# phandasm/waveform

Hardware: AMD Instinct MI355X
Metric: spectra/sec at FFT=4096, batch=4096 streams; achieved HBM GB/s vs peak (higher is better)
Workload: dtype f32

## Files before the change

waveform_amd/csrc/wf_hip_plan.hip:

```cpp
#include <hip/hip_runtime.h>

#include <algorithm>
#include <cmath>
#include <cstdarg>
#include <cstdio>
#include <cstdlib>
#include <cstring>
#include <new>
#include <string>
#include <vector>

#include "wf_hip_internal.hpp"
#include "wf_geometry.hpp"

namespace wf::host {

thread_local std::string g_create_error;

int fail(wf_hip *h, int code, const char *fmt, ...)
{
    char buf[512];
    va_list ap;
    va_start(ap, fmt);
    vsnprintf(buf, sizeof(buf), fmt, ap);
// ... 111 lines not shown
    h->out_ch = h->tab.output_channels;
    h->disp_ch = h->tab.display_channels;
    h->num_bars = (uint32_t)h->tab.num_bars;
    h->ring_cap = next_pow2(ring_frames ? std::max(ring_frames, h->N) : std::max(2 * h->N, 4096u));
    h->plan = wf::plan_transform(cfg, ov);
    h->tick.mr.passes = h->plan.passes;
    std::copy(h->plan.radix, h->plan.radix + 4, h->tick.mr.radix);
    h->wave = cfg.waveform != 0;
    h->meter = cfg.meter != 0;
    if(h->wave) {
        h->M = h->N;
        h->ring_cap = next_pow2(std::max(ring_frames, 2 * (wave_samples + h->N)));
    }
    uint32_t pad = h->ring_cap >= 65536u ? 16448u : 0u;
#ifdef WF_DEV_BUILD
    if(const char *e = std::getenv("WF_HIP_RING_PAD"))
        pad = (uint32_t)std::strtoul(e, nullptr, 10) & ~3u;
#endif
    h->ring_stride = h->ring_cap + pad;
    if(h->wave)
        fill_wave_args(h, wave_samples);
    return WF_HIP_OK;
}

int open_device(wf_hip *h, int *cu_count)
{
    WF_HIP_TRY(h, hipSetDevice(h->device));
    hipDeviceProp_t prop{};
    WF_HIP_TRY(h, hipGetDeviceProperties(&prop, h->device));
    if(std::strncmp(prop.gcnArchName, "gfx950", 6) != 0)
        return fail(h, WF_HIP_ERR_NO_DEVICE, "device %d is %s; this library contains gfx950 code only", h->device, prop.gcnArchName);
    *cu_count = prop.multiProcessorCount;
    WF_HIP_TRY(h, hipStreamCreateWithFlags(&h->stream, hipStreamNonBlocking));
    WF_HIP_TRY(h, hipEventCreate(&h->ev0));
    WF_HIP_TRY(h, hipEventCreate(&h->ev1));
    return WF_HIP_OK;
}

size_t spectra(const wf_hip *h) { return (size_t)h->n_streams * h->cap_ch; }

int finish_create(wf_hip *h)
{
    WF_TRY_RC(wf_hip_reset(h, 0, h->n_streams));
    WF_HIP_TRY(h, hipStreamSynchronize(h->stream));
    return WF_HIP_OK;
}

int create_waveform(wf_hip *h)
{
    WF_TRY_RC(dev_alloc(h, &h->d_cend, (size_t)h->n_streams));
    WF_TRY_RC(dev_alloc(h, &h->d_wts, (size_t)h->n_streams));
    WF_TRY_RC(dev_alloc(h, &h->d_decibels, (size_t)h->n_streams * h->out_ch * h->M));
    WF_TRY_RC(dev_alloc(h, &h->d_flags, (size_t)h->n_streams));
    h->kernel_name = "waveform_tick_kernel";
    return finish_create(h);
}

int create_meter(wf_hip *h)
{
    WF_TRY_RC(dev_alloc(h, &h->d_mend, (size_t)h->n_streams));
    WF_TRY_RC(dev_alloc(h, &h->d_meter_buf, spectra(h)));
    WF_TRY_RC(dev_alloc(h, &h->d_meter_val, spectra(h)));
    WF_TRY_RC(dev_alloc(h, &h->d_flags, (size_t)h->n_streams));
    WF_TRY_RC(dev_alloc(h, &h->d_bars, spectra(h)));
    h->kernel_name = "meter_tick_kernel";
    fill_meter_args(h);
    return finish_create(h);
}

int alloc_spectrum_state(wf_hip *h)
{
    const wf_config *cfg = &h->cfg;
    WF_TRY_RC(dev_alloc(h, &h->d_tsmooth, spectra(h) * h->M));
    WF_TRY_RC(dev_alloc(h, &h->d_decibels, (size_t)h->n_streams * h->out_ch * h->M));
    h->flag_bufs = h->plan.want_split ? 3 : 1;
    WF_TRY_RC(dev_alloc(h, &h->d_flags, (size_t)h->flag_bufs * h->n_streams));
    if(h->plan.want_split)
        WF_TRY_RC(dev_alloc(h, &h->d_verdict, 3 * spectra(h)));
    if(h->num_bars)
        WF_TRY_RC(dev_alloc(h, &h->d_bars, (size_t)h->n_streams * h->disp_ch * h->num_bars));
    if(h->num_bars && cfg->mirror_freq_axis)
        WF_TRY_RC(dev_alloc(h, &h->d_bars_pre, (size_t)h->n_streams * h->disp_ch));
#ifdef WF_PHASE_TIMING
    WF_TRY_RC(dev_alloc(h, &h->tick.phase_clock, spectra(h) * 16));
#endif
    if(!cfg->vertices)
        return WF_HIP_OK;
    if(cfg->vertices > 3u || (cfg->vertices == 3u && (!cfg->bars || cfg->step_width < 1 || cfg->step_gap < 0)) || (cfg->vertices == 2u && cfg->bars) ||
       (!cfg->bars && !cfg->curve))
        return fail(h, WF_HIP_ERR_INVALID, "cfg.vertices: 1 needs bars or curve, 2 the curve, 3 bars with step_width >= 1 and step_gap >= 0");
    wf::VertexTables vtab;
    if(h->num_bars != 0)
        wf::build_vertex_tables(*cfg, (int)h->num_bars, vtab);
    if(h->num_bars != 0 && vtab.per_row > 0) {
        const size_t rows = (size_t)h->n_streams * h->disp_ch;
        float *d_cap_xy = nullptr;
        WF_TRY_RC(dev_alloc(h, &h->d_vert_counts, rows));
        WF_HIP_TRY(h, hipMemsetAsync(h->d_vert_counts, 0, rows * sizeof(uint32_t), h->stream));
        WF_TRY_RC(dev_alloc(h, &h->d_verts, rows * vtab.per_row));
        WF_HIP_TRY(h, hipMemsetAsync(h->d_verts, 0, rows * vtab.per_row * sizeof(wf::f4), h->stream));
        WF_TRY_RC(upload(h, &d_cap_xy, vtab.cap_xy));
        WF_HIP_TRY(h, hipStreamSynchronize(h->stream));
        fill_vertex_args(h, vtab, d_cap_xy);
    }
    return WF_HIP_OK;
}

int upload_window_tables(wf_hip *h)
{
    const std::vector<float> ones_m(h->M, 1.0f);
    const float in_scale = h->plan.in_scale;
    std::vector<float> win_dev(h->N, in_scale);
    for(size_t i = 0; i < h->tab.window.size() && i < win_dev.size(); ++i)
        win_dev[i] = h->tab.window[i] * in_scale;
    WF_TRY_RC(upload(h, &h->tick.window, win_dev));
    WF_TRY_RC(upload(h, &h->tick.slope, h->tab.slope.empty() ? ones_m : h->tab.slope));
    WF_HIP_TRY(h, hipStreamSynchronize(h->stream));
    return upload(h, &h->tick.rolloff, h->tab.rolloff);
}

struct DisplayRoom {
    bool own_kernel;
    size_t lds_floats;
    int threads, points, kmax;
};

void fill_bar_scalars(wf_hip *h)
{
    wf::BarArgs &b = h->tick.bar;
    b.gauss_radius = h->tab.gauss_radius;
    b.entries = (int)h->tab.bar_coef.size();
    b.num_bars = (int)h->num_bars;
    b.mirror = h->cfg.mirror_freq_axis ? 1 : 0;
    b.border_top = h->tab.border_top;
    b.border_bottom = h->tab.border_bottom;
    b.ceiling = (float)h->cfg.ceiling_db;
    b.dbrange = (float)(h->cfg.ceiling_db - h->cfg.floor_db);
    b.inv_dbrange = 1.0f / b.dbrange;
    b.lerp_mixed = ((b.border_top <= 0 && b.border_bottom >= 0) || (b.border_top >= 0 && b.border_bottom <= 0)) ? 1 : 0;
    b.disp_ch = h->disp_ch;
}

int plan_curve(wf_hip *h, DisplayRoom &room)
{
    const wf_config *cfg = &h->cfg;
    wf::BarArgs &b = h->tick.bar;
    wf::CurveLaneTables cl;
    bool both = !cfg->stereo && cfg->capture_channels == 2 && !room.own_kernel && !h->plan.want_split && !h->plan.blu && h->N >= 1024u;
#ifdef WF_DEV_BUILD
    both = both && std::getenv("WF_HIP_TLDS") == nullptr;
    if(const char *e = std::getenv("WF_HIP_CURVE_BOTH"))
        both = both && e[0] != '0';
#endif
    b.both_subs = both ? 1 : 0;
    if(both)
        room.threads *= 2;
    if(!wf::curve_lanes(h->tab, *cfg, room.threads, room.kmax, cl))
        return fail(h, WF_HIP_ERR_INVALID, "curve display: no point table for width %u at fft_size %u", cfg->width, h->N);
    b.out_steps = cl.steps;
    b.curve = cl.x.empty() ? 1 : 2;
    b.stream_steps = (cl.steps > room.kmax || room.own_kernel) ? 1 : 0;
    WF_TRY_RC(upload(h, &b.cur_coef, cl.coef));
    WF_TRY_RC(upload(h, &b.cur_base, cl.base));
    WF_TRY_RC(upload(h, &b.cur_x, cl.x));
    WF_HIP_TRY(h, hipStreamSynchronize(h->stream));
    return WF_HIP_OK;
}
// ... 511 lines not shown
```

waveform_amd/csrc/wf_kernels.hpp:

```cpp
#pragma once
#include <hip/hip_runtime.h>
#include "wf_geometry.hpp"
#include "wf_tick_phases.hpp"
#include "wf_mixed.hpp"
#include "wf_hip.h"
#ifndef WF_EXP_NO_TAIL
#define WF_EXP_NO_TAIL 0
#endif
#include "wf_dev_guard.hpp"

namespace wf {

template<class G> __device__ __forceinline__ void spectrum_sync()
{
    if constexpr(G::T > 64)
        __syncthreads();
    else
        __builtin_amdgcn_wave_barrier();
}

template<int BYTES> __device__ __forceinline__ void lds_dma_copy(const void *src, void *lds_dst, int wave, int n_waves, int lane)
{
    constexpr int W = (BYTES % 1024 == 0) ? 16 : 4;
    constexpr int PER = 64 * W;
    static_assert(BYTES % PER == 0, "table size must be a multiple of the request size");
    constexpr int CALLS = BYTES / PER;
#pragma unroll
    for(int c = 0; c < CALLS; ++c) {
        if((c % n_waves) == wave) {
            const char *g = static_cast<const char *>(src) + c * PER + lane * W;
            char *l = static_cast<char *>(lds_dst) + c * PER;
            if constexpr(W == 16)
                __builtin_amdgcn_global_load_lds((const __attribute__((address_space(1))) void *)g,
                                                 (__attribute__((address_space(3))) void *)l, 16, 0, 0);
            else
                __builtin_amdgcn_global_load_lds((const __attribute__((address_space(1))) void *)g,
                                                 (__attribute__((address_space(3))) void *)l, 4, 0, 0);
        }
    }
}

template<class G, int SPW> constexpr size_t tick_lds_bytes()
{
    return (size_t)SPW * G::LDS_CF * sizeof(cf) + (size_t)G::R2 * G::R3 * sizeof(cf) + 2 * (size_t)SPW * (G::T / 64) * sizeof(int) + 16;
}

#ifndef WF_TRACK
#define WF_TRACK 1
#endif
#ifndef WF_DEFER_STATE
#define WF_DEFER_STATE 0
#endif
#ifndef WF_WPS_SMALL
#define WF_WPS_SMALL 4
#endif
#ifndef WF_WPS_2048_BLU
#define WF_WPS_2048_BLU 4
#endif
#ifndef WF_MR_FIXED_PLANS
#define WF_MR_FIXED_PLANS 1
#endif
#ifndef WF_WPS_2048_MRS
#define WF_WPS_2048_MRS 5
#endif
#ifndef WF_WPS_2048
#define WF_WPS_2048 3
#endif
#ifndef WF_WPS_512
#define WF_WPS_512 6
#endif
#ifndef WF_WPS_LARGE
#define WF_WPS_LARGE 4
#endif
#define WF_WAVES_PER_SIMD(G) ((G::P > 16) ? 2 : (G::P > 8 && G::T <= 64) ? WF_WPS_2048 : (G::P <= 4) ? WF_WPS_512 : (G::P <= 8) ? WF_WPS_SMALL : WF_WPS_LARGE)

#ifdef WF_PHASE_TIMING
#define WF_STAMP(i)                                                                      \
    do {                                                                                 \
        if(threadIdx.x == 0 && a.phase_clock)                                            \
            a.phase_clock[(size_t)blockIdx.x * 16 + (i)] = __builtin_readcyclecounter(); \
    } while(0)
#define WF_STAMP_HWID()                                                                                          \
    do {                                                                                                         \
        if(threadIdx.x == 0 && a.phase_clock) {                                                                  \
            a.phase_clock[(size_t)blockIdx.x * 16 + 11] = __builtin_amdgcn_s_getreg((32 - 1) << 11 | 0 << 6 | 4); \
            a.phase_clock[(size_t)blockIdx.x * 16 + 12] = __builtin_amdgcn_s_getreg((32 - 1) << 11 | 0 << 6 | 20); \
        }                                                                                                        \
    } while(0)
#elif defined(WF_EXP_CUT_AT)
#define WF_STAMP(i)         \
    do {                    \
        if((i) == WF_EXP_CUT_AT) \
            return;         \
    } while(0)
#define WF_STAMP_HWID()
#else
#define WF_STAMP(i)
#define WF_STAMP_HWID()
#endif

struct Variant {
    int spw = 2;
    bool aligned = false;
    bool split = false;
    int dec = 0;
    bool tlds = false;
    bool blu = false;
    bool both = false;
    bool mr = false;
    bool mrs = false;
    bool mir = false;
    int disp = 0;
    int plan = 0;
};
template<class G, Variant V> constexpr int tick_waves_per_simd()
{
    return V.mrs ? WF_WPS_2048_MRS : (V.blu && G::P > 8 && G::T <= 64) ? WF_WPS_2048_BLU : WF_WAVES_PER_SIMD(G);
}
template<class G, Variant V>
__global__ __launch_bounds__(V.spw * G::T, (tick_waves_per_simd<G, V>())) void spectrum_tick_kernel(const TickArgs a)
{
#ifdef WF_PHASE_TIMING
    const unsigned long long clock_entry = __builtin_readcyclecounter();
#endif
    constexpr int SPW = V.spw, DEC = V.dec, DISP = V.disp, PLAN = V.plan;
    constexpr bool ALIGNED = V.aligned, SPLIT = V.split, TLDS = V.tlds, BLU = V.blu, BOTH = V.both, MR = V.mr, MRS = V.mrs, MIR = V.mir;
    static_assert(!MRS || (MR && G::T <= 256 && G::P > 8), "the small-radix instantiation belongs to the containers of one, two and four wavefronts");
    static_assert(!BOTH || (SPW == 2 && !SPLIT && DEC == 0 && !BLU), "shared curve row: two spectra per workgroup, power-of-two sizes");
    static_assert(!BLU || (DEC == 0 && !TLDS && !ALIGNED), "Bluestein path: scalar fetch, no decimation, no staged tables");
    static_assert(!MR || BLU, "the mixed-radix transform (wf_mixed.hpp) runs inside the Bluestein instantiation's fetch and epilogue");
    static_assert(!TLDS || (SPW == 2 && !SPLIT && DEC == 0 && (size_t)SPW * G::LDS_CF * sizeof(cf) >= 2u * G::N * sizeof(float)),
                  "staged tables: window + pass-1 twiddles must fit the workgroup's exchange buffers");
    static_assert(!SPLIT || SPW == 1, "split mode: one spectrum per workgroup");
    static_assert(DEC == 0 || (!SPLIT && G::T == 64 && (G::R1 >> DEC) >= 1 && (G::M >> DEC) >= 64), "decimated path: one-wavefront geometry");
    constexpr bool MIRROR = MIR || SPLIT;
    constexpr int MO_C = G::M >> DEC;
    using RG = RowG<DEC ? MO_C / 4 : G::T, DEC ? 4 : G::P>;
    constexpr int RP = RG::P;
    const int MO = BLU ? (int)a.row_bins : MO_C;
    const int NB = MO;
    extern __shared__ __attribute__((aligned(16))) unsigned char smem_raw[];
    constexpr int T = G::T, P = G::P, WPS = G::T / 64;
    const int tid = (int)threadIdx.x;
    const int sub = __builtin_amdgcn_readfirstlane(tid / T);
    const int t = tid % T;
    const int lane = tid & 63;
    const int wave_in_block = tid >> 6;
    constexpr bool PS_OK = !BLU && DEC == 0 && !BOTH;
    static_assert(DISP != 1 || PS_OK, "the prefix-sum bars belong to the power-of-two kernels");
    const bool has_display = DISP == 1 ? true : DISP == 2 ? false : (a.bar.out != nullptr);
#define WF_PS_MODE (PS_OK && (DISP == 1 || (DISP == 0 && a.bar.out != nullptr && a.bar.ps_lanes > 0)))
#define WF_PS_FINISHER (WF_PS_MODE && (t >> 6) == 0)
    const uint32_t n_spec = (a.stream_base + a.stream_count) * a.cap_ch;
    uint32_t spec_raw = a.stream_base * a.cap_ch + blockIdx.x * SPW + (uint32_t)sub;
    if constexpr(SPLIT) {
        if(a.split_ch != 0xffffffffu)
            spec_raw = 2u * (a.stream_base + blockIdx.x) + a.split_ch;
    }
    const bool active = spec_raw < n_spec;
    const uint32_t spec = active ? spec_raw : n_spec - 1;
    const uint32_t cap_shift = a.cap_ch - 1;
    const uint32_t stream = spec >> cap_shift;
    const uint32_t ch = spec & cap_shift;
    const bool stereo = (a.mode & WF_MODE_STEREO) != 0;
    const bool mono_mix = (a.mode & WF_MODE_MONO_MIX) != 0;
    const uint32_t wpos = a.wpos[stream];
    const uint32_t sflags = a.stream_flags[stream];
    const float vol_comp = a.vol_comp_stream ? a.vol_comp_stream[stream] : a.vol_comp;
    uint32_t vin0 = 0, vin1 = 0;
    if constexpr(SPLIT) {
        vin0 = a.verdict_in[2u * stream];
        vin1 = a.verdict_in[2u * stream + 1u];
    }

    const int lds_cf = MR ? a.mr.lds_cf : (int)G::LDS_CF;
    cf *lds = reinterpret_cast<cf *>(smem_raw) + (size_t)sub * lds_cf;
    cf *tw2_lds = reinterpret_cast<cf *>(smem_raw) + (size_t)SPW * lds_cf;
    int *facts = reinterpret_cast<int *>(tw2_lds + G::R2 * G::R3);
    int *arrivals = facts + 2 * SPW * WPS + sub;
    const float *x = a.ring + (size_t)spec * a.ring_stride;
    const uint32_t delay = a.delay + (a.delay_stream ? a.delay_stream[stream] : 0u);
    const uint32_t start = (wpos - delay - (BLU ? a.blu_n : (uint32_t)(G::N >> DEC))) & a.ring_mask;
    float *ts = a.tsmooth + (size_t)spec * MO;
    float *rows = a.decibels + (size_t)stream * a.out_ch * MO;
    const bool row_thread = DEC == 0 || t < RG::T;

    const bool paused = (sflags & WF_STREAM_PAUSED) != 0;
    const bool hidden = (sflags & (WF_STREAM_HIDDEN | WF_STREAM_PAUSED)) != 0;
    const bool was_silent = (sflags & WF_STREAM_LAST_SILENT) != 0 || paused;

    WF_STAMP(0);
    WF_STAMP_HWID();
#ifdef WF_PHASE_TIMING
    if(DISP == 2 && threadIdx.x == 0 && a.phase_clock)
        a.phase_clock[(size_t)blockIdx.x * 16 + 14] = clock_entry;
#endif
    P1Regs<G> r1;
    bool nz = false;
    float mr_touch[2] = {0.0f, 0.0f};
    MrOps<G> mr_ops;
    constexpr bool MR_EARLY = BLU && MR && WF_MR_PREFETCH && G::T == 64;
    if constexpr(BLU && MR) {
        if(active)
            nz = mr_fetch<G>(a, t, x, start, lds) && !hidden;
        if constexpr(MR_EARLY)
            mr_ops_request<G, true, false>(a, t, ts, mr_ops);
        if(G::T > 64 && active && 16 * t < MO) {
            mr_touch[0] = (a.mode & WF_MODE_TSMOOTH) ? ts[16 * t] : 0.0f;
            mr_touch[1] = a.slope[16 * t];
        }
    } else if constexpr(BLU) {
        if(active)
            nz = (blu_table_via_lds<G>() ? p1_fetch_blu<G>(a, t, x, start, r1) : p1_fetch_blu_direct<G>(a, t, x, start, r1)) && !hidden;
    } else if(active)
        nz = p1_fetch<G, ALIGNED, DEC, TLDS>(a, t, x, start, r1) && !hidden;
    if constexpr(TLDS) {
        lds_dma_copy<G::N * (int)sizeof(float)>(a.window, smem_raw, wave_in_block, T * SPW / 64, lane);
        lds_dma_copy<G::M * (int)sizeof(cf)>(a.tw1, smem_raw + G::N * sizeof(float), wave_in_block, T * SPW / 64, lane);
    }
    if constexpr(BLU && !MR && blu_table_via_lds<G>())
        blu_table_to_lds(a, smem_raw, wave_in_block, T * SPW / 64, lane);
    lds_dma_copy<G::R2 * G::R3 * (int)sizeof(cf)>(a.tw2, tw2_lds, wave_in_block, T * SPW / 64, lane);
    BarPre bar_pre_early{0, 0, 1, 0, 0, 0, -1};
    if constexpr(!(BLU && !MR))
        if constexpr(DISP == 0)
            bar_pre_early = bars_preload<G, true, PS_OK>(a.bar, t);
    const bool wave_nz = __any(nz) != 0;
    WF_STAMP(1);
    bool wave_below = true;
    if(active && !hidden && !wave_nz) {
        if(!SPLIT && (WF_TRACK && a.bars_only != nullptr) && a.bars_only->use_verdict)
            wave_below = a.bars_only->row_verdict[(size_t)(spec - (stereo ? 0u : ch)) * WPS + (wave_in_block - sub * WPS)] == 0u;
        else
            wave_below = __all(!row_thread || row_all_below<RG, BLU>(rows + (size_t)(stereo ? ch : 0u) * MO, t, a.silent_floor, NB)) != 0;
    }

    bool nz0 = wave_nz, nz1 = false, below0 = wave_below, below1 = true;
    if(lane == 0)
        facts[wave_in_block] = (wave_nz ? 1 : 0) | (wave_below ? 2 : 0);
    if(T > 64 && t == 0)
        *arrivals = 0;
    if(PS_OK && tid < 2)
        facts[2 * SPW * WPS + 2 + tid] = 0;
    __syncthreads();
    if constexpr(SPLIT) {
        int orf = 0;
#pragma unroll
        for(int w = 0; w < WPS; ++w)
            orf |= facts[w];
        const bool nz_own = (orf & 1) != 0;
        bool nz_other = false;
        if(!nz_own && !hidden) {
            const float *xo = a.ring + (size_t)(spec ^ 1u) * a.ring_stride;
            uint32_t acc = 0;
            const uint32_t wlen = BLU ? a.blu_n : (uint32_t)G::N;
            for(uint32_t i = (uint32_t)tid; i < wlen; i += (uint32_t)T)
                acc |= f32_bits(xo[(start + i) & a.ring_mask]);
            const bool w_nz = __any((acc & 0x7fffffffu) != 0) != 0;
            if(lane == 0)
                facts[WPS + wave_in_block] = w_nz ? 1 : 0;
            __syncthreads();
            int o2 = 0;
#pragma unroll
            for(int w = 0; w < WPS; ++w)
                o2 |= facts[WPS + w];
            nz_other = o2 != 0;
        }
        nz0 = ch == 0 ? nz_own : nz_other;
        nz1 = ch == 0 ? nz_other : nz_own;
        below0 = vin0 == 0u;
        below1 = stereo ? (vin1 == 0u) : (vin0 == 0u);
    } else if(T > 64 || a.cap_ch > 1) {
        const int sb0 = (sub - (int)ch) * WPS;
        int or0 = 0, and0 = 3, or1 = 0, and1 = 3;
#pragma unroll
        for(int w = 0; w < WPS; ++w) {
            const int f0 = facts[sb0 + w];
            or0 |= f0;
            and0 &= f0;
            if(a.cap_ch > 1) {
                const int f1 = facts[sb0 + WPS + w];
                or1 |= f1;
                and1 &= f1;
            }
        }
        nz0 = (or0 & 1) != 0;
        below0 = (and0 & 2) != 0;
        nz1 = (or1 & 1) != 0;
        below1 = (and1 & 2) != 0;
    }
    StreamPlan plan = plan_stream(was_silent, a.cap_ch, stereo, nz0, nz1, below0, below1);
    const uint32_t fft_n = BLU ? a.blu_n : (uint32_t)(G::N >> DEC);
    const bool underflow = (!(sflags & WF_STREAM_WRAPPED) && (wpos - fft_n) < delay) || (sflags & WF_STREAM_STARVED) != 0;
    if(underflow) {
        plan.process0 = plan.process1 = false;
        plan.last_silent = was_silent;
    }
    const bool process = active && !hidden && (ch == 0 ? plan.process0 : plan.process1);
    const bool do_db = active && !hidden && !plan.last_silent;

    cf v[P];
    float mag[RP];
    WF_STAMP(2);
    P4Regs<G> r4;
    if constexpr(BLU && MR) {
// ... 272 lines not shown
            exceeds = (ch == 0 ? vin0 : vin1) != 0u;
        if(__any(exceeds) && lane == 0)
            atomicOr(a.verdict_out + spec, 1u);
        if(tid == 0)
            a.verdict_clear[spec] = 0u;
    }

#ifndef WF_TAIL_PRIO
#define WF_TAIL_PRIO 0
#endif
    if(!BLU && MIRROR && has_display && a.bar.out2_n > 0 && active && ch < a.bar.disp_ch) {
        const bool have_row_ = do_db && !(mono_mix && ch == 1);
        const bool reset_ = hidden && !was_silent && ch < (stereo ? 2u : 1u);
        if(!have_row_ && !reset_) {
            const float *bo = a.bar.out + ((size_t)stream * a.bar.disp_ch + ch) * a.bar.num_bars;
            const int n = a.bar.num_bars * ((a.out_ch > a.cap_ch) ? 2 : 1);
            for(int i = t; i < n; i += T) {
                const float v = bo[i];
#pragma unroll
                for(int j = 0; j < 8; ++j)
                    if(j < a.bar.out2_n)
                        const_cast<float *>(bo)[(long long)i + a.bar.out2_delta[j]] = v;
            }
        }
    }
    if(has_display && !WF_EXP_NO_TAIL) {
        if(WF_TAIL_PRIO > 0)
            __builtin_amdgcn_s_setprio(WF_TAIL_PRIO);
        constexpr bool both = BOTH;
        float *dbl = both ? reinterpret_cast<float *>(smem_raw) : reinterpret_cast<float *>(lds);
        auto row_sync = [&] {
            if(both)
                __syncthreads();
            else
                spectrum_sync<G>();
        };
        if(count_arrivals) {
            while(__hip_atomic_load(arrivals, WF_ARRIVE_ORDER_ACQ, __HIP_MEMORY_SCOPE_WORKGROUP) < WPS)
                __builtin_amdgcn_s_sleep(1);
            asm volatile("" ::: "memory");
        } else if(!(mono_mix && !SPLIT))
            row_sync();
        if constexpr(PS_OK) {
            if(WF_PS_MODE) {
                const bool ps_finisher = (t >> 6) == 0;
                WF_STAMP(12);
                if(have_row)
                    ps_park<RG>(dbl, MO, t, d);
                WF_STAMP(14);
                int *parked = facts + 2 * SPW * WPS + 2 + sub;
                if constexpr(T > 64) {
                    if(lane == 0)
                        __hip_atomic_fetch_add(parked, 1, __ATOMIC_RELEASE, __HIP_MEMORY_SCOPE_WORKGROUP);
                    if(ps_finisher) {
                        while(__hip_atomic_load(parked, __ATOMIC_ACQUIRE, __HIP_MEMORY_SCOPE_WORKGROUP) < WPS)
                            __builtin_amdgcn_s_sleep(1);
                    }
                } else
                    __builtin_amdgcn_wave_barrier();
                WF_STAMP(15);
                if(ps_finisher) {
                    float *out0 = a.bar.out + ((size_t)stream * a.bar.disp_ch + ch) * a.bar.num_bars;
                    const BarArgs bar_row = [&] { BarArgs b = a.bar; if(!MIRROR) b.out2_n = 0; if(b.pre_out) b.pre_out += (size_t)stream * a.bar.disp_ch + ch; return b; }();
                    ps_finish<G, RG>(bar_row, bar_entries, dbl, MO, lane, have_row, out0, dup_row ? out0 + a.bar.num_bars : nullptr);
                }
                WF_STAMP(13);
                return;
            }
        }
        if constexpr(DISP == 1)
            return;
        if(have_row && row_thread)
            store_row<RG, BLU>(dbl, t, d, NB);
        if(a.bar.curve == 2 && have_row && t == 0)
            dbl[MO] = dbl[MO + 1] = 0.0f;
        if((BLU && !MR) || !a.bar.piece_mode)
            row_sync();
        float *out0 = a.bar.out + ((size_t)stream * a.bar.disp_ch + ch) * a.bar.num_bars;
        float *out1 = dup_row ? out0 + a.bar.num_bars : nullptr;
#ifdef WF_PHASE_TIMING
        BarArgs bar_args = a.bar;
        if(bar_args.pre_out)
            bar_args.pre_out += (size_t)stream * a.bar.disp_ch + (BOTH ? 0u : ch);
        bar_args.clk = (a.phase_clock && threadIdx.x == 0) ? a.phase_clock + (size_t)blockIdx.x * 16 : nullptr;
        WF_STAMP(12);
#else
        const BarArgs bar_row = [&] {
            BarArgs b = a.bar;
            if(BLU || !MIRROR)
                b.out2_n = 0;
            if(b.pre_out)
                b.pre_out += (size_t)stream * a.bar.disp_ch + (BOTH ? 0u : ch);
            return b;
        }();
        const BarArgs &bar_args = bar_row;
#endif
        OutVals<G> ov;
        bool pending = true;
        if constexpr(BOTH) {
            {
                constexpr int TT = 2 * T;
                float *row0 = a.bar.out + (size_t)stream * a.bar.disp_ch * a.bar.num_bars;
                if(a.bar.stream_steps) {
                    curve_row_stream<G, TT>(bar_args, do_db, dbl, dbl, tid, row0, nullptr, [] { __syncthreads(); });
                } else {
                    if(a.bar.curve == 2)
                        curve_row_catrom<G, TT>(bar_args, do_db, dbl, tid, ov);
                    else
                        curve_row<G, TT>(bar_args, do_db, dbl, tid, ov);
                    outputs_finish<G, TT>(bar_args, do_db, ov, dbl, tid, row0, nullptr, [] { __syncthreads(); });
                }
                pending = false;
            }
        }
        if(pending && !both) {
            if(a.bar.stream_steps) {
                curve_row_stream<G>(bar_args, have_row, dbl, dbl, t, out0, out1, [] { spectrum_sync<G>(); });
                pending = false;
            } else if(a.bar.curve == 2)
                curve_row_catrom<G>(bar_args, have_row, dbl, t, ov);
            else if(a.bar.curve)
                curve_row<G>(bar_args, have_row, dbl, t, ov);
            else
                pending = bars_reduce_row<G, !(BLU && !MR)>(
                    bar_args, (BLU && !MR) ? bars_preload<G, false, false>(a.bar, t) : bar_pre_early, bar_entries, have_row, dbl, dbl + MO, t, out0, out1, ov, [] { spectrum_sync<G>(); },
                    [](float v, int m) { return v + __shfl_xor(v, m, 64); }, arrivals, count_arrivals ? 2 * WPS : WPS);
            if(pending)
                outputs_finish<G>(bar_args, have_row, ov, dbl, t, out0, out1, [] { spectrum_sync<G>(); });
        }
    }
    WF_STAMP(13);
#undef WF_PS_MODE
#undef WF_PS_FINISHER
}

}
```

waveform_amd/csrc/wf_tick_phases.hpp:

```cpp
#pragma once
#include "wf_fft_core.hpp"

namespace wf {

enum : uint32_t {
    WF_MODE_TSMOOTH = 1u << 0,
    WF_MODE_FAST_PEAKS = 1u << 1,
    WF_MODE_STEREO = 1u << 2,
    WF_MODE_NORMALIZE = 1u << 3,
    WF_MODE_ROLLOFF = 1u << 4,
    WF_MODE_SLOPE = 1u << 5,
    WF_MODE_WINDOW = 1u << 6,
    WF_MODE_MONO_MIX = 1u << 7,
};

enum : uint32_t {
    WF_STREAM_LAST_SILENT = 1u << 0,
    WF_STREAM_HIDDEN = 1u << 1,
    WF_STREAM_TIMEOUT = 1u << 2,
    WF_STREAM_PAUSED = 1u << 4,
    WF_STREAM_STARVED = 1u << 5,
    WF_STREAM_WRAPPED = 1u << 3,
};

struct BarArgs {
    const float *coef;
    const int *bin;
    const int *off;
    const int *count;
    const int *chunk;
    const int *big_task;
    const int *big_bar_task;
    int big_num_tasks;
    const float *lane_coef;
    const int *lane_base;
    const int *bar_seg;
    const int *seg_group;
    const int *lead_bar;
    const int *lead_end;
    int wave_local;
    int piece_mode;
    const float *ps_tab;
    int ps_lanes;
    int num_segs;
    int lane_blocks;
    const float *cur_coef;
    const int *cur_base;
    const float *cur_x;
    int curve;
    int out_steps;
    int both_subs;
    int stream_steps;
    const float *gauss;
    const float *gauss_wsum;
    int gauss_radius;
    int stage_off;
#ifdef WF_PHASE_TIMING
    unsigned long long *clk;
#endif
    float *out;
    float *pre_out;
    int out2_n;
    long long out2_delta[8];
    int num_bars;
    int num_chunks;
    int entries;
    int lanes_per_bar;
    int mirror;
    float border_top, border_bottom;
    float ceiling, dbrange;
    float inv_dbrange;
    int lerp_mixed;
    uint32_t disp_ch;
};

#ifdef WF_PHASE_TIMING
#define WF_BAR_STAMP(i) do { if(t == 0 && b.clk) b.clk[i] = __builtin_readcyclecounter(); } while(0)
#else
#define WF_BAR_STAMP(i)
#endif

struct BarsOnlyState {
    uint32_t *row_verdict;
    const float *stale_row;
    uint32_t use_verdict;
};

constexpr int MR_MAX_PASSES = 4;
struct MrPlan {
    int passes;
    int radix[MR_MAX_PASSES];
    int tw_off[MR_MAX_PASSES];
    const cf *wp;
    const cf *tw;
    int half, s3, lds_cf;
};
WF_DEV int mr_z_addr(const MrPlan &p, int k) { return (k & 3) * p.s3 + (k >> 2); }

struct TickArgs {
    const float *ring;
    const uint32_t *wpos;
    uint32_t ring_mask;
    uint32_t ring_cap;
    uint32_t ring_stride;
    uint32_t delay;
    const uint32_t *delay_stream;
    const float *window;
    const cf *tw1;
    const cf *tw2;
    const cf *tws;
    const float *slope;
    const float *rolloff;
    float *tsmooth;
    float *decibels;
    uint32_t *stream_flags;
    uint32_t *flags_out;
    const uint32_t *verdict_in;
    uint32_t *verdict_out;
    uint32_t *verdict_clear;
    float half_coef;
    float slope_step;
    float g, g2;
    float vol_comp;
    const float *vol_comp_stream;
    float db_min;
    float silent_floor;
    uint32_t n_streams;
    uint32_t stream_base, stream_count;
    uint32_t cap_ch;
    uint32_t out_ch;
    uint32_t mode;
    uint32_t skip_decibels;
    uint32_t split_ch;
    const BarsOnlyState *bars_only;
    const float *stale_row;
    const cf *blu_q;
    const cf *blu_qr;
    const cf *blu_w;
    MrPlan mr;
    uint32_t big_c, big_r;
    uint32_t big_rs;
    const cf *big_wc;
    const cf *blu_a;
    const cf *blu_b;
    uint32_t blu_n;
    uint32_t row_bins;
    const cf *big_z;
    const cf *big_tws;
    const cf *big_tw;
    uint32_t *big_nz_out;
    const uint32_t *big_nz;
    uint32_t big_m, big_l;
    BarArgs bar;
    unsigned long long *phase_clock;
};

WF_DEV f4 ld4(const float *p) { return *reinterpret_cast<const f4 *>(p); }
WF_DEV f2 ld2(const float *p) { return *reinterpret_cast<const f2 *>(p); }
WF_DEV void st4(float *p, f4 v) { *reinterpret_cast<f4 *>(p) = v; }
#ifndef WF_SLOPE_LINEAR
#define WF_SLOPE_LINEAR 1
#endif
#ifndef WF_BAR_COEF_EARLY
#define WF_BAR_COEF_EARLY 1
#endif
#ifndef WF_NT_ROWS
#define WF_NT_ROWS true
#endif
#ifndef WF_NT_STATE
#define WF_NT_STATE 1
#endif
#ifndef WF_NT_SMP
#define WF_NT_SMP 0
#endif
#ifndef WF_NT_STATE_LD
#define WF_NT_STATE_LD 1
#endif
#if defined(__HIPCC__)
WF_DEV f4 ld4_nt(const float *p)
{
    typedef float v4f __attribute__((ext_vector_type(4)));
    const v4f v = __builtin_nontemporal_load(reinterpret_cast<const v4f *>(p));
    return f4{v.x, v.y, v.z, v.w};
}
WF_DEV void st4_nt(float *p, f4 v)
{
    typedef float v4f __attribute__((ext_vector_type(4)));
    __builtin_nontemporal_store(v4f{v.x, v.y, v.z, v.w}, reinterpret_cast<v4f *>(p));
}
#else
WF_DEV f4 ld4_nt(const float *p) { return ld4(p); }
WF_DEV void st4_nt(float *p, f4 v) { st4(p, v); }
#endif

WF_DEV f4 ld_state(const float *p) { return WF_NT_STATE_LD ? ld4_nt(p) : ld4(p); }
WF_DEV void st_state(float *p, f4 v)
{
    if(WF_NT_STATE)
        st4_nt(p, v);
    else
        st4(p, v);
}

WF_DEV float mul_unfused(float a, float b)
{
#pragma clang fp contract(off)
    return a * b;
}
WF_DEV float add_unfused(float a, float b)
{
#pragma clang fp contract(off)
    return a + b;
}
WF_DEV float meter_ema(float g, float old, float g2, float cur)
{
#pragma clang fp contract(off)
    const float x = g * old;
    const float y = g2 * cur;
    return x + y;
}

#ifndef WF_EMA_GENERIC
#define WF_EMA_GENERIC 1
#endif
WF_DEV float spectrum_ema(float g, float old, float g2, float cur)
{
#if WF_EMA_GENERIC
    return meter_ema(g, old, g2, cur);
#else
    return fmaf(g, old, g2 * cur);
#endif
}

#if defined(__HIPCC__)
WF_DEV void wait_vmem_all() { __builtin_amdgcn_s_waitcnt(0x0F70); }
WF_DEV void wave_fence() { __builtin_amdgcn_wave_barrier(); }
WF_DEV float wave_shfl_down(float v, int d) { return __shfl_down(v, d, 64); }
WF_DEV float seg_prefix_scan(float v, uint32_t info)
// ... 8 lines not shown
    WF_SCAN_STEP(0x114, 0xf, 2)
    WF_SCAN_STEP(0x118, 0xf, 3)
    WF_SCAN_STEP(0x142, 0xa, 4)
    WF_SCAN_STEP(0x143, 0xc, 5)
#undef WF_SCAN_STEP
    return v;
}
#ifndef WF_ARRIVE_RELAXED
#define WF_ARRIVE_RELAXED 0
#endif
#define WF_ARRIVE_ORDER_REL (WF_ARRIVE_RELAXED ? __ATOMIC_RELAXED : __ATOMIC_RELEASE)
#define WF_ARRIVE_ORDER_ACQ (WF_ARRIVE_RELAXED ? __ATOMIC_RELAXED : __ATOMIC_ACQUIRE)
WF_DEV int wave_arrive(int *counter, int lane)
{
    int old = 0;
    asm volatile("" ::: "memory");
    if(lane == 0)
        old = __hip_atomic_fetch_add(counter, 1, WF_ARRIVE_RELAXED ? __ATOMIC_RELAXED : __ATOMIC_ACQ_REL, __HIP_MEMORY_SCOPE_WORKGROUP);
    old = __builtin_amdgcn_readfirstlane(old);
    asm volatile("" ::: "memory");
    return old;
}
#else
WF_DEV void wait_vmem_all() {}
WF_DEV void wave_fence() {}
WF_DEV float wave_shfl_down(float v, int) { return v; }
WF_DEV float seg_prefix_scan(float v, uint32_t) { return v; }
WF_DEV int wave_arrive(int *counter, int) { return __atomic_fetch_add(counter, 1, __ATOMIC_ACQ_REL); }
#endif

#ifndef WF_LDS_TRACE
#define WF_LDS_TRACE(idx, bytes, is_write)
#endif
WF_DEV cf lds_ld2(const cf *lds, int idx) { WF_LDS_TRACE(idx, 8, 0); return lds[idx]; }
WF_DEV void lds_st2(cf *lds, int idx, cf a) { WF_LDS_TRACE(idx, 8, 1); lds[idx] = a; }
WF_DEV f4 lds_ld4(const cf *lds, int idx) { WF_LDS_TRACE(idx, 16, 0); return *reinterpret_cast<const f4 *>(lds + idx); }
WF_DEV void lds_st4(cf *lds, int idx, cf a, cf b) { WF_LDS_TRACE(idx, 16, 1); *reinterpret_cast<f4 *>(lds + idx) = f4{a.x, a.y, b.x, b.y}; }


WF_DEV uint32_t f32_bits(float v)
{
#if defined(__HIPCC__)
    return __float_as_uint(v);
#else
    uint32_t u;
    __builtin_memcpy(&u, &v, 4);
    return u;
#endif
}

#ifndef WF_FAST_DB
#define WF_FAST_DB 1
#endif
WF_DEV float dbfs(float mag, float db_min)
{
#if defined(__HIPCC__) && WF_FAST_DB
    return fmaxf(__builtin_amdgcn_logf(mag) * 6.02059991327962390f, db_min);
#else
    return (mag > 0.0f) ? 20.0f * log10f(mag) : db_min;
#endif
}

#ifndef WF_FAST_SQRT
#define WF_FAST_SQRT 1
#endif
WF_DEV float mag2(float xr, float xi)
{
    const float s = fmaf(xi, xi, xr * xr);
#if defined(__HIPCC__) && WF_FAST_SQRT
#if defined(WF_MAG_SAFE)
    if(__builtin_expect(s < 0x1p-100f, 0)) {
        const float a = xr * 0x1p64f, b = xi * 0x1p64f;
        return __builtin_amdgcn_sqrtf(fmaf(b, b, a * a)) * 0x1p-64f;
    }
#endif
    return __builtin_amdgcn_sqrtf(s);
#else
    return sqrtf(s);
#endif
}

#ifndef WF_PREFETCH_STATE
#define WF_PREFETCH_STATE -1
#endif
template<class G> struct Policy {
    static_assert(G::P <= 32, "the phase functions keep a thread's operands in registers: at most 32 points per thread (two waves per SIMD)");
    static constexpr int MODE = (WF_PREFETCH_STATE >= 0) ? WF_PREFETCH_STATE : (G::P <= 8 ? 1 : 0);
    static constexpr bool PREFETCH_STATE = (MODE == 1 || MODE == 3);
    static constexpr bool PREFETCH_SLOPE = (MODE == 1 || MODE == 3);
    static constexpr bool TOUCH_STATE = (MODE == 2);
    static constexpr bool PREFETCH_LATE = (MODE == 3);
    static constexpr bool SLOPE_LINEAR = (WF_SLOPE_LINEAR != 0) && MODE == 0;
    static constexpr bool BAR_COEF_EARLY = (WF_BAR_COEF_EARLY != 0) && SLOPE_LINEAR && G::T >= 128;
};
#ifndef WF_TW1_POW2
#define WF_TW1_POW2 1
#endif
constexpr bool tw1_row_loaded(int k1) { return !WF_TW1_POW2 || (k1 & (k1 - 1)) == 0; }

template<class G> struct P1Regs {
    float smp[G::R1][2 * G::B1];
    float win[G::R1][2 * G::B1];
    float tw1[G::R1][2 * G::B1];
    cf wb[4];
};

template<class G> WF_DEV void p1_load_window(const TickArgs &a, int t, int j, float (&win)[2 * G::B1])
{
    constexpr int B1 = G::B1, M1 = G::M1;
    const uint32_t s0 = 2u * (uint32_t)(j * M1 + B1 * t);
    if(B1 == 2) {
        const f4 w = ld4(a.window + s0);
        win[0] = w.x; win[1] = w.y; win[2 * B1 - 2] = w.z; win[2 * B1 - 1] = w.w;
    } else {
        const f2 w = ld2(a.window + s0);
        win[0] = w.x; win[1] = w.y;
    }
}
template<class G> WF_DEV void p1_load_tw1(const TickArgs &a, int t, int k1, float (&tw1)[2 * G::B1])
{
    constexpr int B1 = G::B1, M1 = G::M1;
    const float *tw = reinterpret_cast<const float *>(a.tw1 + k1 * M1 + B1 * t);
    if(B1 == 2) {
        const f4 w = ld4(tw);
        tw1[0] = w.x; tw1[1] = w.y; tw1[2 * B1 - 2] = w.z; tw1[2 * B1 - 1] = w.w;
    } else {
        const f2 w = ld2(tw);
        tw1[0] = w.x; tw1[1] = w.y;
    }
}

template<class G, bool ALIGNED, int DEC = 0, bool TLDS = false>
WF_DEV bool p1_fetch(const TickArgs &a, int t, const float *x, uint32_t start, P1Regs<G> &r)
{
    constexpr int R1 = G::R1, B1 = G::B1, M1 = G::M1;
    constexpr int RV = R1 >> DEC;
    static_assert(RV >= 1, "zero-padding leaves at least one row of samples per thread");
    WF_UNROLL
    for(int j = 0; j < R1; ++j) {
        const uint32_t s0 = 2u * (uint32_t)(j * M1 + B1 * t);
        if(j >= RV) {
            WF_UNROLL
            for(int e = 0; e < 2 * B1; ++e) {
                r.smp[j][e] = 0.0f;
                r.win[j][e] = 0.0f;
            }
        } else if(ALIGNED) {
            if(B1 == 2) {
                const f4 q = WF_NT_SMP ? ld4_nt(x + ((start + s0) & a.ring_mask)) : ld4(x + ((start + s0) & a.ring_mask));
                r.smp[j][0] = q.x; r.smp[j][1] = q.y; r.smp[j][2 * B1 - 2] = q.z; r.smp[j][2 * B1 - 1] = q.w;
            } else {
                const f2 q = ld2(x + ((start + s0) & a.ring_mask));
                r.smp[j][0] = q.x; r.smp[j][1] = q.y;
            }
        } else {
            WF_UNROLL
            for(int e = 0; e < 2 * B1; ++e)
                r.smp[j][e] = *(x + ((start + s0 + (uint32_t)e) & a.ring_mask));
        }
    }
    WF_UNROLL
    for(int j = 0; j < R1; ++j) {
        if(j < RV && !TLDS)
            p1_load_window<G>(a, t, j, r.win[j]);
        if(j >= 1 && !TLDS && tw1_row_loaded(j))
            p1_load_tw1<G>(a, t, j, r.tw1[j]);
    }
    if(DEC == 0) {
        const f4 wa = ld4(reinterpret_cast<const float *>(a.tws + 4 * t));
        const f4 wc = ld4(reinterpret_cast<const float *>(a.tws + 4 * t + 2));
        r.wb[0] = cf{wa.x, wa.y}; r.wb[1] = cf{wa.z, wa.w}; r.wb[2] = cf{wc.x, wc.y}; r.wb[3] = cf{wc.z, wc.w};
    } else {
        WF_UNROLL
        for(int i = 0; i < 4; ++i) {
            const int k = ((4 * t + i) << DEC) & (G::M - 1);
            const f2 w = ld2(reinterpret_cast<const float *>(a.tws + k));
            r.wb[i] = cf{w.x, w.y};
        }
    }
    uint32_t acc = 0;
    WF_UNROLL
    for(int j = 0; j < R1; ++j) {
        WF_UNROLL
        for(int e = 0; e < 2 * B1; ++e)
            acc |= f32_bits(r.smp[j][e]);
    }
    return (acc & 0x7fffffffu) != 0;
}

template<class G>
WF_DEV void p1_window_dft(P1Regs<G> &r, cf (&o)[G::R1][G::B1])
{
    constexpr int R1 = G::R1, B1 = G::B1;
    cf u[B1][R1];
    WF_UNROLL
    for(int j = 0; j < R1; ++j) {
        WF_UNROLL
        for(int e = 0; e < 2 * B1; ++e)
            r.smp[j][e] *= r.win[j][e];
        WF_UNROLL
        for(int b = 0; b < B1; ++b)
            u[b][j] = cf{r.smp[j][2 * b], r.smp[j][2 * b + 1]};
    }
    WF_UNROLL
    for(int b = 0; b < B1; ++b)
        dft_dif<R1>(u[b]);
    constexpr int LB = ilog2(R1);
    WF_UNROLL
    for(int k1 = 0; k1 < R1; ++k1) {
        if(k1 >= 1 && !tw1_row_loaded(k1)) {
            const int lo = k1 & -k1, hi = k1 - lo;
            WF_UNROLL
            for(int b = 0; b < B1; ++b) {
                const cf w = cmul(cf{r.tw1[hi][2 * b], r.tw1[hi][2 * b + 1]}, cf{r.tw1[lo][2 * b], r.tw1[lo][2 * b + 1]});
                r.tw1[k1][2 * b] = w.x;
                r.tw1[k1][2 * b + 1] = w.y;
            }
        }
        WF_UNROLL
        for(int b = 0; b < B1; ++b)
            o[k1][b] = (k1 == 0) ? u[b][0] : cmul(u[b][brev(k1, LB)], cf{r.tw1[k1][2 * b], r.tw1[k1][2 * b + 1]});
    }
}
template<class G> WF_DEV void p1_store(int t, cf *lds, const cf (&o)[G::R1][G::B1])
{
    constexpr int R1 = G::R1, B1 = G::B1;
    const int np = B1 * t;
    WF_UNROLL
    for(int k1 = 0; k1 < R1; ++k1) {
        if(B1 == 2)
            lds_st4(lds, ex1_addr<G>(k1, np), o[k1][0], o[k1][B1 - 1]);
        else
            lds_st2(lds, ex1_addr<G>(k1, np), o[k1][0]);
    }
}
template<class G>
WF_DEV void p1_window_pass1(const TickArgs &a, int t, P1Regs<G> &r, cf *lds)
{
    (void)a;
    cf o[G::R1][G::B1];
    p1_window_dft<G>(r, o);
    p1_store<G>(t, lds, o);
}
template<class G> WF_DEV void p1_tables_from_lds(int t, const cf *tab, P1Regs<G> &r)
{
    constexpr int R1 = G::R1, B1 = G::B1, M1 = G::M1, M = G::M;
    WF_UNROLL
    for(int j = 0; j < R1; ++j) {
        if(B1 == 2) {
            const f4 w = lds_ld4(tab, j * M1 + B1 * t);
            r.win[j][0] = w.x; r.win[j][1] = w.y; r.win[j][2 * B1 - 2] = w.z; r.win[j][2 * B1 - 1] = w.w;
            if(j >= 1) {
                const f4 q = lds_ld4(tab, M + j * M1 + B1 * t);
                r.tw1[j][0] = q.x; r.tw1[j][1] = q.y; r.tw1[j][2 * B1 - 2] = q.z; r.tw1[j][2 * B1 - 1] = q.w;
            }
        } else {
            const cf w = lds_ld2(tab, j * M1 + t);
            r.win[j][0] = w.x; r.win[j][1] = w.y;
            if(j >= 1) {
                const cf q = lds_ld2(tab, M + j * M1 + t);
                r.tw1[j][0] = q.x; r.tw1[j][1] = q.y;
            }
        }
    }
}

template<class G> struct P4Regs {
    float st[Policy<G>::PREFETCH_STATE ? G::P : 1];
    float sl[Policy<G>::PREFETCH_SLOPE ? G::P : 1];
    float touch[2];
// ... 1396 lines not shown
```

Before: 145.2 million.

## Issue table loads and tw2 LDS copy before ring sample fetch

Result: no change. 144.5 million (-0.5%).

```diff
diff --git a/waveform_amd/csrc/wf_hip_plan.hip b/waveform_amd/csrc/wf_hip_plan.hip
--- a/waveform_amd/csrc/wf_hip_plan.hip
+++ b/waveform_amd/csrc/wf_hip_plan.hip
@@ -217,7 +217,7 @@
     if(h->num_bars && cfg->mirror_freq_axis)
         WF_TRY_RC(dev_alloc(h, &h->d_bars_pre, (size_t)h->n_streams * h->disp_ch));
 #ifdef WF_PHASE_TIMING
-    WF_TRY_RC(dev_alloc(h, &h->tick.phase_clock, spectra(h) * 16));
+    WF_TRY_RC(dev_alloc(h, &h->tick.phase_clock, spectra(h) * WF_STAMP_SLOTS));
 #endif
     if(!cfg->vertices)
         return WF_HIP_OK;
diff --git a/waveform_amd/csrc/wf_kernels.hpp b/waveform_amd/csrc/wf_kernels.hpp
--- a/waveform_amd/csrc/wf_kernels.hpp
+++ b/waveform_amd/csrc/wf_kernels.hpp
@@ -78,13 +78,13 @@
 #define WF_STAMP(i)                                                                      \
     do {                                                                                 \
         if(threadIdx.x == 0 && a.phase_clock)                                            \
-            a.phase_clock[(size_t)blockIdx.x * 16 + (i)] = __builtin_readcyclecounter(); \
+            a.phase_clock[wf_stamp_block * WF_STAMP_SLOTS + (i)] = __builtin_readcyclecounter(); \
     } while(0)
 #define WF_STAMP_HWID()                                                                                          \
     do {                                                                                                         \
         if(threadIdx.x == 0 && a.phase_clock) {                                                                  \
-            a.phase_clock[(size_t)blockIdx.x * 16 + 11] = __builtin_amdgcn_s_getreg((32 - 1) << 11 | 0 << 6 | 4); \
-            a.phase_clock[(size_t)blockIdx.x * 16 + 12] = __builtin_amdgcn_s_getreg((32 - 1) << 11 | 0 << 6 | 20); \
+            a.phase_clock[wf_stamp_block * WF_STAMP_SLOTS + 11] = __builtin_amdgcn_s_getreg((32 - 1) << 11 | 0 << 6 | 4); \
+            a.phase_clock[wf_stamp_block * WF_STAMP_SLOTS + WF_STAMP_XCC] = __builtin_amdgcn_s_getreg((32 - 1) << 11 | 0 << 6 | 20); \
         }                                                                                                        \
     } while(0)
 #elif defined(WF_EXP_CUT_AT)
@@ -124,6 +124,9 @@
     const unsigned long long clock_entry = __builtin_readcyclecounter();
 #endif
     constexpr int SPW = V.spw, DEC = V.dec, DISP = V.disp, PLAN = V.plan;
+#ifdef WF_PHASE_TIMING
+    const size_t wf_stamp_block = (size_t)a.stream_base * a.cap_ch / SPW + blockIdx.x;
+#endif
     constexpr bool ALIGNED = V.aligned, SPLIT = V.split, TLDS = V.tlds, BLU = V.blu, BOTH = V.both, MR = V.mr, MRS = V.mrs, MIR = V.mir;
     static_assert(!MRS || (MR && G::T <= 256 && G::P > 8), "the small-radix instantiation belongs to the containers of one, two and four wavefronts");
     static_assert(!BOTH || (SPW == 2 && !SPLIT && DEC == 0 && !BLU), "shared curve row: two spectra per workgroup, power-of-two sizes");
@@ -166,7 +169,16 @@
     const bool mono_mix = (a.mode & WF_MODE_MONO_MIX) != 0;
     const uint32_t wpos = a.wpos[stream];
     const uint32_t sflags = a.stream_flags[stream];
-    const float vol_comp = a.vol_comp_stream ? a.vol_comp_stream[stream] : a.vol_comp;
+    constexpr bool TF = Policy<G>::tables_first(DISP, BOTH) && !BLU && !TLDS && DEC == 0;
+    float vol_comp;
+    uint32_t delay_s = 0;
+    if constexpr(TF) {
+        const uint32_t dw = *(a.delay_stream ? a.delay_stream + stream : a.wpos + stream);
+        const uint32_t vw = *(a.vol_comp_stream ? reinterpret_cast<const uint32_t *>(a.vol_comp_stream) + stream : a.wpos + stream);
+        delay_s = a.delay_stream ? dw : 0u;
+        vol_comp = a.vol_comp_stream ? __uint_as_float(vw) : a.vol_comp;
+    } else
+        vol_comp = a.vol_comp_stream ? a.vol_comp_stream[stream] : a.vol_comp;
     uint32_t vin0 = 0, vin1 = 0;
     if constexpr(SPLIT) {
         vin0 = a.verdict_in[2u * stream];
@@ -179,7 +191,7 @@
     int *facts = reinterpret_cast<int *>(tw2_lds + G::R2 * G::R3);
     int *arrivals = facts + 2 * SPW * WPS + sub;
     const float *x = a.ring + (size_t)spec * a.ring_stride;
-    const uint32_t delay = a.delay + (a.delay_stream ? a.delay_stream[stream] : 0u);
+    const uint32_t delay = a.delay + (TF ? delay_s : (a.delay_stream ? a.delay_stream[stream] : 0u));
     const uint32_t start = (wpos - delay - (BLU ? a.blu_n : (uint32_t)(G::N >> DEC))) & a.ring_mask;
     float *ts = a.tsmooth + (size_t)spec * MO;
     float *rows = a.decibels + (size_t)stream * a.out_ch * MO;
@@ -192,8 +204,8 @@
     WF_STAMP(0);
     WF_STAMP_HWID();
 #ifdef WF_PHASE_TIMING
-    if(DISP == 2 && threadIdx.x == 0 && a.phase_clock)
-        a.phase_clock[(size_t)blockIdx.x * 16 + 14] = clock_entry;
+    if(threadIdx.x == 0 && a.phase_clock)
+        a.phase_clock[wf_stamp_block * WF_STAMP_SLOTS + WF_STAMP_ENTRY] = clock_entry;
 #endif
     P1Regs<G> r1;
     bool nz = false;
@@ -212,6 +224,14 @@
     } else if constexpr(BLU) {
         if(active)
             nz = (blu_table_via_lds<G>() ? p1_fetch_blu<G>(a, t, x, start, r1) : p1_fetch_blu_direct<G>(a, t, x, start, r1)) && !hidden;
+    } else if constexpr(TF) {
+        p1_fetch_tables<G, DEC, TLDS>(a, t, r1);
+        lds_dma_copy<G::R2 * G::R3 * (int)sizeof(cf)>(a.tw2, tw2_lds, wave_in_block, T * SPW / 64, lane);
+        __builtin_amdgcn_sched_barrier(0);
+        if(active) {
+            p1_fetch_ring<G, ALIGNED, DEC>(a, t, x, start, r1);
+            nz = p1_nonzero<G>(r1) && !hidden;
+        }
     } else if(active)
         nz = p1_fetch<G, ALIGNED, DEC, TLDS>(a, t, x, start, r1) && !hidden;
     if constexpr(TLDS) {
@@ -220,7 +240,8 @@
     }
     if constexpr(BLU && !MR && blu_table_via_lds<G>())
         blu_table_to_lds(a, smem_raw, wave_in_block, T * SPW / 64, lane);
-    lds_dma_copy<G::R2 * G::R3 * (int)sizeof(cf)>(a.tw2, tw2_lds, wave_in_block, T * SPW / 64, lane);
+    if constexpr(!TF)
+        lds_dma_copy<G::R2 * G::R3 * (int)sizeof(cf)>(a.tw2, tw2_lds, wave_in_block, T * SPW / 64, lane);
     BarPre bar_pre_early{0, 0, 1, 0, 0, 0, -1};
     if constexpr(!(BLU && !MR))
         if constexpr(DISP == 0)
@@ -659,7 +680,7 @@
         BarArgs bar_args = a.bar;
         if(bar_args.pre_out)
             bar_args.pre_out += (size_t)stream * a.bar.disp_ch + (BOTH ? 0u : ch);
-        bar_args.clk = (a.phase_clock && threadIdx.x == 0) ? a.phase_clock + (size_t)blockIdx.x * 16 : nullptr;
+        bar_args.clk = (a.phase_clock && threadIdx.x == 0) ? a.phase_clock + wf_stamp_block * WF_STAMP_SLOTS : nullptr;
         WF_STAMP(12);
 #else
         const BarArgs bar_row = [&] {
diff --git a/waveform_amd/csrc/wf_tick_phases.hpp b/waveform_amd/csrc/wf_tick_phases.hpp
--- a/waveform_amd/csrc/wf_tick_phases.hpp
+++ b/waveform_amd/csrc/wf_tick_phases.hpp
@@ -1,4 +1,6 @@
 #pragma once
+#include <cstddef>
+
 #include "wf_fft_core.hpp"
 
 namespace wf {
@@ -74,6 +76,9 @@
     uint32_t disp_ch;
 };
 
+#define WF_STAMP_SLOTS 18
+#define WF_STAMP_ENTRY 16
+#define WF_STAMP_XCC 17
 #ifdef WF_PHASE_TIMING
 #define WF_BAR_STAMP(i) do { if(t == 0 && b.clk) b.clk[i] = __builtin_readcyclecounter(); } while(0)
 #else
@@ -98,62 +103,64 @@
 WF_DEV int mr_z_addr(const MrPlan &p, int k) { return (k & 3) * p.s3 + (k >> 2); }
 
 struct TickArgs {
+    uint32_t stream_base, stream_count;
+    uint32_t cap_ch;
+    uint32_t mode;
+    uint32_t delay;
+    uint32_t ring_mask;
+    uint32_t ring_stride;
+    float vol_comp;
+    const uint32_t *wpos;
+    uint32_t *stream_flags;
+    const uint32_t *delay_stream;
+    const float *vol_comp_stream;
     const float *ring;
-    const uint32_t *wpos;
-    uint32_t ring_mask;
-    uint32_t ring_cap;
-    uint32_t ring_stride;
-    uint32_t delay;
-    const uint32_t *delay_stream;
     const float *window;
     const cf *tw1;
     const cf *tw2;
     const cf *tws;
-    const float *slope;
-    const float *rolloff;
     float *tsmooth;
     float *decibels;
-    uint32_t *stream_flags;
+    const float *slope;
+    float half_coef;
+    float slope_step;
+    float g, g2;
+    float db_min;
+    float silent_floor;
+    uint32_t out_ch;
+    uint32_t skip_decibels;
+    uint32_t n_streams;
+    uint32_t ring_cap;
+    uint32_t split_ch;
+    uint32_t row_bins;
+    const float *rolloff;
     uint32_t *flags_out;
     const uint32_t *verdict_in;
     uint32_t *verdict_out;
     uint32_t *verdict_clear;
-    float half_coef;
-    float slope_step;
-    float g, g2;
-    float vol_comp;
-    const float *vol_comp_stream;
-    float db_min;
-    float silent_floor;
-    uint32_t n_streams;
-    uint32_t stream_base, stream_count;
-    uint32_t cap_ch;
-    uint32_t out_ch;
-    uint32_t mode;
-    uint32_t skip_decibels;
-    uint32_t split_ch;
     const BarsOnlyState *bars_only;
     const float *stale_row;
+    BarArgs bar;
+    MrPlan mr;
     const cf *blu_q;
     const cf *blu_qr;
     const cf *blu_w;
-    MrPlan mr;
+    const cf *blu_a;
+    const cf *blu_b;
+    uint32_t blu_n;
     uint32_t big_c, big_r;
     uint32_t big_rs;
     const cf *big_wc;
-    const cf *blu_a;
-    const cf *blu_b;
-    uint32_t blu_n;
-    uint32_t row_bins;
     const cf *big_z;
     const cf *big_tws;
     const cf *big_tw;
     uint32_t *big_nz_out;
     const uint32_t *big_nz;
     uint32_t big_m, big_l;
-    BarArgs bar;
     unsigned long long *phase_clock;
 };
+static_assert(offsetof(TickArgs, wpos) == 32 && offsetof(TickArgs, vol_comp_stream) == 56, "the per-stream words' block is the first 64 bytes");
+static_assert(offsetof(TickArgs, ring) == 64 && offsetof(TickArgs, slope) == 120 && offsetof(TickArgs, half_coef) == 128, "the burst's pointers are the second 64 bytes");
 
 WF_DEV f4 ld4(const float *p) { return *reinterpret_cast<const f4 *>(p); }
 WF_DEV f2 ld2(const float *p) { return *reinterpret_cast<const f2 *>(p); }
@@ -328,6 +335,9 @@
 
 #ifndef WF_PREFETCH_STATE
 #define WF_PREFETCH_STATE -1
+#endif
+#ifndef WF_TABLES_FIRST
+#define WF_TABLES_FIRST 7
 #endif
 template<class G> struct Policy {
     static_assert(G::P <= 32, "the phase functions keep a thread's operands in registers: at most 32 points per thread (two waves per SIMD)");
@@ -338,6 +348,12 @@
     static constexpr bool PREFETCH_LATE = (MODE == 3);
     static constexpr bool SLOPE_LINEAR = (WF_SLOPE_LINEAR != 0) && MODE == 0;
     static constexpr bool BAR_COEF_EARLY = (WF_BAR_COEF_EARLY != 0) && SLOPE_LINEAR && G::T >= 128;
+    static constexpr bool tables_first(int disp, bool both)
+    {
+        return (G::N == 4096 && disp == 1 && (WF_TABLES_FIRST & 1)) || (G::N == 8192 && disp == 1 && (WF_TABLES_FIRST & 2)) ||
+               (G::N == 4096 && disp == 0 && both && (WF_TABLES_FIRST & 4)) || (G::N == 2048 && disp == 1 && (WF_TABLES_FIRST & 8)) ||
+               (G::N == 16384 && disp == 1 && (WF_TABLES_FIRST & 16)) || (G::N == 4096 && disp == 0 && !both && (WF_TABLES_FIRST & 32));
+    }
 };
 #ifndef WF_TW1_POW2
 #define WF_TW1_POW2 1
@@ -376,8 +392,8 @@
     }
 }
 
-template<class G, bool ALIGNED, int DEC = 0, bool TLDS = false>
-WF_DEV bool p1_fetch(const TickArgs &a, int t, const float *x, uint32_t start, P1Regs<G> &r)
+template<class G, bool ALIGNED, int DEC = 0>
+WF_DEV void p1_fetch_ring(const TickArgs &a, int t, const float *x, uint32_t start, P1Regs<G> &r)
 {
     constexpr int R1 = G::R1, B1 = G::B1, M1 = G::M1;
     constexpr int RV = R1 >> DEC;
@@ -405,6 +421,24 @@
                 r.smp[j][e] = *(x + ((start + s0 + (uint32_t)e) & a.ring_mask));
         }
     }
+}
+template<class G> WF_DEV bool p1_nonzero(const P1Regs<G> &r)
+{
+    constexpr int R1 = G::R1, B1 = G::B1;
+    uint32_t acc = 0;
+    WF_UNROLL
+    for(int j = 0; j < R1; ++j) {
+        WF_UNROLL
+        for(int e = 0; e < 2 * B1; ++e)
+            acc |= f32_bits(r.smp[j][e]);
+    }
+    return (acc & 0x7fffffffu) != 0;
+}
+template<class G, int DEC = 0, bool TLDS = false>
+WF_DEV void p1_fetch_tables(const TickArgs &a, int t, P1Regs<G> &r)
+{
+    constexpr int R1 = G::R1;
+    constexpr int RV = R1 >> DEC;
     WF_UNROLL
     for(int j = 0; j < R1; ++j) {
         if(j < RV && !TLDS)
@@ -424,14 +458,13 @@
             r.wb[i] = cf{w.x, w.y};
         }
     }
-    uint32_t acc = 0;
-    WF_UNROLL
-    for(int j = 0; j < R1; ++j) {
-        WF_UNROLL
-        for(int e = 0; e < 2 * B1; ++e)
-            acc |= f32_bits(r.smp[j][e]);
-    }
-    return (acc & 0x7fffffffu) != 0;
+}
+template<class G, bool ALIGNED, int DEC = 0, bool TLDS = false>
+WF_DEV bool p1_fetch(const TickArgs &a, int t, const float *x, uint32_t start, P1Regs<G> &r)
+{
+    p1_fetch_ring<G, ALIGNED, DEC>(a, t, x, start, r);
+    p1_fetch_tables<G, DEC, TLDS>(a, t, r);
+    return p1_nonzero<G>(r);
 }
 
 template<class G>
```
